# pashtari/factorizer

Measured on AMD Instinct MI355X. Metric: volumes/sec fwd+bwd, Swin Factorizer 128^3, higher is better.
Workload: dtype f32

## Files before the change

factorizer_amd/csrc/gemm.hip:

```cpp
#include "gemm_bx.h"
#include "finish.h"

namespace fz {

__device__ __forceinline__ float half_sum32(float v) {
  v += dpp_take<0xB1, 0xf>(v);
  v += dpp_take<0x4E, 0xf>(v);
  v += dpp_take<0x141, 0xf>(v);
  v += dpp_take<0x140, 0xf>(v);
  v += dpp_take<0x142, 0xa>(v);
  return v;
}

template <int NACC, bool GADD, bool GADD_LDS = false, typename AT = float>
__device__ __forceinline__ void lnbwd_block(const GemmArgsT<AT>& p, const f32x16 (&acc)[NACC], int b, int64_t ncol,
                                            bool col_ok, int lane, int wave, float* red ,
                                            int64_t part_row, const float* g_lds ,
                                            const float* gadd_lds = nullptr ) {
  const int h = lane >> 5;
  const int64_t nc = col_ok ? ncol : 0;
  const unsigned lane_off = (unsigned)(4 * h) * (unsigned)p.Ncol + (unsigned)nc;
  const int64_t sample = (int64_t)b * 32 * p.Ncol;
  const float* sp = p.lnb_stats + (int64_t)b * 2 * p.Ncol;
  float mu[NACC], rs[NACC];
// ... 2540 lines not shown
        s2[e] += src[(MB * NACC * 16 + NACC + e) * 64];
      }
    }
  }

  float mu_d[NACC], rstd[NACC];
  if (PRO == PRO_LN) {
#pragma unroll
    for (int e = 0; e < NACC; ++e) {
      const float t1 = s1[e] + __shfl_xor(s1[e], 32, 64);
      const float t2 = s2[e] + __shfl_xor(s2[e], 32, 64);
      const float inv = 1.0f / (float)p.Cin;
      const float md = t1 * inv;
      float var = t2 * inv - md * md;
      var = var > 0.f ? var : 0.f;
      mu_d[e] = md;
      rstd[e] = 1.0f / sqrtf(var + p.ln_eps);
    }
    if (p.stats_out != nullptr && by == 0 && h == 0 && col_ok) {
      float mean[NACC];
#pragma unroll
      for (int e = 0; e < NACC; ++e) mean[e] = shift[e] + mu_d[e];
      float* so = p.stats_out + (int64_t)b * 2 * p.Vin;
      vstore<NACC>(so + col_off, mean);
      vstore<NACC>(so + p.Vin + col_off, rstd);
    }
  }
  if (!col_ok) return;
  const int64_t ncol = (LOADER == LOAD_S2D) ? n0 + 2 * j : col_off;
#pragma unroll
  for (int mb = 0; mb < MB; ++mb) {
    if (PRO == PRO_LN) {
#pragma unroll
      for (int r = 0; r < 16; ++r) {
        const int rl = (r & 3) + 8 * (r >> 2) + 4 * h;
        const float sw = sW[mb * 32 + rl];
#pragma unroll
        for (int q = 0; q < NACC; ++q) acc[mb][q][r] = rstd[q] * (acc[mb][q][r] - mu_d[q] * sw);
      }
    }
    store_block<NACC, EPI, LOADER == LOAD_S2D>(p, acc[mb], b, m0 + mb * 32, ncol, h,
                                                PRO == PRO_LN ? tW + mb * 32 : nullptr);
  }
}

}

using namespace fz;

static std::atomic<int> g_bx_on{-1};
static int knob_pos(const fz::EnvKnob& k, int dflt) { return k.set && k.val > 0 ? k.val : dflt; }
static int knob_mlp_wg_wgs() { return knob_pos(FZ_KNOB("FZ_MLP_WG_WGS"), 512); }
static int knob_gemm_dw_wgs() { return knob_pos(FZ_KNOB("FZ_GEMM_DW_WGS"), 512); }
static int knob_chain64_p512() { return knob_pos(FZ_KNOB("FZ_CHAIN64_P512"), 1) == 1; }
static int knob_res_prefetch() { return knob_pos(FZ_KNOB("FZ_RES_PREFETCH"), 1) == 1; }
static int knob_p32() { return knob_pos(FZ_KNOB("FZ_GEMM_P32"), 1) == 1; }
static int knob_p32_wgs() { return knob_pos(FZ_KNOB("FZ_GEMM_P32_WGS"), 512); }
static int knob_head_fwd() { const auto& k = FZ_KNOB("FZ_HEAD_FWD"); return k.set ? k.val : 1; }
static int knob_chain_wgb() { const auto& k = FZ_KNOB("FZ_CHAIN_WGB"); return k.set ? k.val : 1; }
static int knob_chain_fwd_bx() { const auto& k = FZ_KNOB("FZ_CHAIN_FWD_BX"); return k.set ? k.val : 1; }
static int knob_mlp_wgs(int dflt) { return knob_pos(FZ_KNOB("FZ_MLP_WGS"), dflt); }

static int gemm_bx_enabled() {
  int v = g_bx_on.load(std::memory_order_relaxed);
  if (v < 0) {
    const char* e = getenv("FZ_GEMM_BX");
    v = e ? (atoi(e) != 0) : 1;
    g_bx_on.store(v, std::memory_order_relaxed);
  }
  return v;
}
extern "C" int fz_gemm_bx_enable(int on) {
  const int prev = gemm_bx_enabled();
  if (on >= 0) g_bx_on.store(on != 0, std::memory_order_relaxed);
  return prev;
}

template <typename AT>
static int gemm_launch(const fz_gemm_desc* d, fz_stream_t stream) {
  if (!d->x[0] || !d->w || !d->y) return fail(FZ_E_ARG, "fz_gemm: null pointer");
  if (d->loader < LOAD_PLAIN || d->loader > LOAD_K3) return fail(FZ_E_ARG, "fz_gemm: bad loader");
  if (d->epilogue < EPI_PLAIN || d->epilogue > EPI_LNBWD) return fail(FZ_E_ARG, "fz_gemm: bad epilogue");
  const bool lnb64 = d->epilogue == EPI_LNBWD && d->M == 64 && d->K == 64 && d->nsrc == 1 && !d->bmul;
  if (d->epilogue == EPI_LNBWD && ((!lnb64 && (d->M != 32 || (d->K != 32 && d->K != 64))) || d->loader != LOAD_PLAIN || !d->lnb_x || !d->lnb_stats ||
                                   !d->lnb_g || !d->lnb_part || d->bias || d->res || d->emul || d->eact || d->ln))
    return fail(FZ_E_UNSUPPORTED, "fz_gemm: LayerNorm-backward epilogue needs M == 32 (K = 32 or 64) or M == K == 64, plain loader");
  if (d->epilogue == EPI_LNBWD && d->Ncol > ((int64_t)1 << 27)) return fail(FZ_E_UNSUPPORTED, "fz_gemm: LayerNorm-backward epilogue: more than 2^27 voxels per sample");
  if (d->B < 0 || d->Cin < 1 || d->M < 1 || d->K < 1) return fail(FZ_E_SHAPE, "fz_gemm: sizes must be positive");
  if ((d->K & 1) && (d->loader != LOAD_PLAIN || d->ln))
    return fail(FZ_E_UNSUPPORTED, "fz_gemm: odd K only with the plain loader and no LayerNorm prologue");
  if (d->loader == LOAD_K3 && (d->epilogue != EPI_PLAIN || d->ln || d->src_mode != 0 || d->nsrc != 1 ||
                               (d->Wi & 3) || d->K != 27 * d->Cin || (d->Cin & 1)))
    return fail(FZ_E_UNSUPPORTED, "fz_gemm: k3 loader needs W % 4 == 0, even Cin, K = 27*Cin, plain epilogue");
  if (d->bmul && (d->loader != LOAD_PLAIN || d->src_mode != 0 || d->nsrc != 1))
    return fail(FZ_E_UNSUPPORTED, "fz_gemm: bmul needs the plain single-source loader");
  if (d->Ncol % 4 != 0 && d->loader != LOAD_S2D) return fail(FZ_E_UNSUPPORTED, "fz_gemm: voxel count must be a multiple of 4");
  if (d->loader == LOAD_S2D && ((d->Wo & 1) || d->epilogue != EPI_PLAIN || d->ln || d->src_mode != 0 || d->nsrc != 1))
    return fail(FZ_E_UNSUPPORTED, "fz_gemm: space-to-depth loader needs even coarse width, plain epilogue");
  if (d->epilogue == EPI_D2S && (d->M % 8 != 0)) return fail(FZ_E_SHAPE, "fz_gemm: depth-to-space rows must be 8*C");
  if (d->nsrc < 1 || d->nsrc > 2 || d->src_mode != 0)
    return fail(FZ_E_UNSUPPORTED, "fz_gemm: one source, or two sources concatenated along channels");
  if (d->bmul && d->bmul_kind != ACT_RELU) return fail(FZ_E_UNSUPPORTED, "fz_gemm: bmul supports the ReLU gate");
  if (d->B == 0) return FZ_OK;
  GemmArgsT<AT> a;
  for (int i = 0; i < 4; ++i) a.x[i] = (const AT*)d->x[i];
  a.nsrc = d->nsrc; a.src_mode = d->src_mode; a.c0 = d->c0 > 0 ? d->c0 : d->Cin; a.Cin = d->Cin;
  a.Vin = d->Vin; a.Di = d->Di; a.Hi = d->Hi; a.Wi = d->Wi; a.bmul = (const AT*)d->bmul; a.bmul_kind = d->bmul_kind;
  a.w = d->w; a.w_t = d->w_t; a.ldw = d->ldw; a.M = d->M; a.K = d->K;
  a.bias = d->bias; a.ln = d->ln; a.ln_g = d->ln_g; a.ln_b = d->ln_b; a.ln_eps = d->ln_eps;
  a.stats_out = d->stats_out; a.bact = d->bact; a.eact = d->eact; a.res = (const AT*)d->res; a.emul = (const AT*)d->emul;
  a.emul_kind = d->emul_kind; a.y = (AT*)d->y; a.Ncol = d->Ncol; a.Ho = d->Ho; a.Wo = d->Wo; a.B = d->B;
  a.dbg = 0; a.tile_map = 1;
  a.ygroups = 0; a.xtiles = 0; a.tune = d->tune;
  a.lnb_x = (const AT*)d->lnb_x; a.lnb_stats = d->lnb_stats; a.lnb_g = d->lnb_g; a.lnb_gadd = (const AT*)d->lnb_gadd; a.lnb_part = d->lnb_part;
  hipStream_t st = (hipStream_t)stream;
  const int mblocks = (d->M + 31) / 32;
  if (lnb64) {
    if (d->Ncol % 4 != 0) return fail(FZ_E_UNSUPPORTED, "fz_gemm: voxel count must be a multiple of 4");
    if (!d->lnb_gadd) return fail(FZ_E_UNSUPPORTED, "fz_gemm: the 64-channel LayerNorm-backward epilogue needs the added gradient");
    ChainArgsT<AT> c = {};
    const int ntiles = (int)fz_mlp_partials(d->B, d->Ncol);
    constexpr int lds64 = (8192 + 8192 + 128 + 64 + 512) * (int)sizeof(float);
    auto kern = products_split(d->products) ? gemm_chain64_kernel<true, AT, true, true> : gemm_chain64_kernel<true, AT, true, false>;
    FZ_HIP_OK(hipFuncSetAttribute(reinterpret_cast<const void*>(kern), hipFuncAttributeMaxDynamicSharedMemorySize, lds64));
    hipLaunchKernelGGL(kern, dim3((unsigned)(ntiles < 512 ? ntiles : 512)), dim3(256), lds64, st, a, c, ntiles);
    FZ_LAUNCH_CHECK();
    return FZ_OK;
  }

  {
    const int bx_on = products_split(d->products);
    const int pro_bx = d->ln ? 1 : (d->bact == ACT_GELU ? 2 : (d->bmul ? 3 : 0));
    const bool one_pro = (d->ln != 0) + (d->bact != 0) + (d->bmul != nullptr) <= 1;
    const int bx_kmin = (sizeof(AT) == 2 && !d->ln && d->bact == 0) ? 32 : 64;
    if (bx_on && one_pro && d->bact != ACT_RELU && d->K >= bx_kmin && d->M >= 32 && (d->loader == LOAD_PLAIN || d->loader == LOAD_S2D) &&
        (d->epilogue == EPI_PLAIN || d->epilogue == EPI_D2S) && !(d->loader == LOAD_S2D && pro_bx) && !(d->epilogue == EPI_D2S && pro_bx))
    {
      const int rc = gemm_bx_launch<AT>(a, d->loader, d->epilogue, pro_bx, stream);
      if (rc != FZ_E_UNSUPPORTED) return rc;
    }
  }

  if (knob_head_fwd() && d->loader == LOAD_PLAIN && d->epilogue == EPI_PLAIN && d->M <= 4 && d->K == 32 && d->Cin == 32 && a.c0 == 32 &&
      !d->ln && !d->bact && !d->eact && !d->res && !d->bmul && !d->emul && !d->w_t && d->ldw == 32 && d->Ncol == d->Vin && d->Ncol % 4 == 0 &&
      d->Ncol / 4 < ((int64_t)1 << 31) && (int64_t)d->B * (d->Ncol / 4) < ((int64_t)1 << 31) && d->stats_out == nullptr)
    return fz_head_fwd(d->x[0], d->w, d->bias, d->y, d->B, d->M, 32, d->Ncol, d->act_dtype, stream);

  if (knob_p32() && d->loader == LOAD_PLAIN && d->epilogue == EPI_PLAIN && d->M <= 32 && d->K == 32 && d->Cin == 32 && (a.c0 & 1) == 0 && d->Vin < ((int64_t)1 << 28) &&
      (int64_t)5 * d->Ncol * (int64_t)sizeof(AT) < ((int64_t)1 << 32)  && !d->res && !d->bmul &&
      !d->emul && d->Ncol % 4 == 0 && d->Ncol == d->Vin && d->B * ((d->Ncol + 127) / 128) >= 4096 && d->B * ((d->Ncol + 127) / 128) < ((int64_t)1 << 30) &&
      !(d->bact && !d->ln) ) {
    const unsigned ntiles = (unsigned)(d->B * ((d->Ncol + 127) / 128));
    const unsigned cap = (unsigned)knob_p32_wgs();
    const unsigned wgs = (ntiles + 3) / 4 < cap ? (ntiles + 3) / 4 : cap;
    const int pf = (d->bact ? 1 : 0) | (d->ln ? 2 : 0);
    dim3 grid(wgs), block(256);
    if (pf == 0) hipLaunchKernelGGL((gemm_p32_kernel<0, AT>), grid, block, 0, st, a, ntiles);
    else if (pf == 2) hipLaunchKernelGGL((gemm_p32_kernel<2, AT>), grid, block, 0, st, a, ntiles);
    else hipLaunchKernelGGL((gemm_p32_kernel<3, AT>), grid, block, 0, st, a, ntiles);
    FZ_LAUNCH_CHECK();
    return FZ_OK;
  }

  int res_maxk = 32;
  if (d->epilogue == EPI_LNBWD) res_maxk = 64;
  const bool stream_small = mblocks == 1 && d->K >= 16 && d->K <= 32 && !d->res && !d->bmul && !d->emul &&
                            d->epilogue == EPI_PLAIN && d->bact == 0;
  if (d->loader == LOAD_PLAIN && d->K <= res_maxk && !stream_small) {
    const int nA = (d->K + 1) / 2;
    int RB = mblocks < 8 ? mblocks : 8;
    while ((size_t)(nA * RB * 64 + 32 * RB) * sizeof(float) > 65536) --RB;
    const size_t lds = (size_t)(nA * RB * 64 + 32 * RB + (d->epilogue == EPI_LNBWD ? 256 : 0)) * sizeof(float);
    const int64_t tiles = (d->Ncol + 511) / 512;
    dim3 grid((unsigned)(tiles * d->B), (unsigned)((mblocks + RB - 1) / RB)), block(256);
#define FZ_RES_PF(NS, E, BM, PFv) hipLaunchKernelGGL((gemm_resident_kernel<NS, E, BM, false, AT, PFv>), grid, block, lds, st, a, RB)
#define FZ_RES(NS, E, BM)                                                  \
  do {                                                                    \
    const int pf = (d->bact ? 1 : 0) | (d->ln ? 2 : 0);                   \
    if (pf == 0) FZ_RES_PF(NS, E, BM, 0);                                 \
    else if (pf == 1) FZ_RES_PF(NS, E, BM, 1);                            \
    else if (pf == 2) FZ_RES_PF(NS, E, BM, 2);                            \
    else FZ_RES_PF(NS, E, BM, 3);                                         \
  } while (0)
    if (d->epilogue == EPI_LNBWD) {
      if (d->bmul) return fail(FZ_E_UNSUPPORTED, "fz_gemm: bmul with LayerNorm-backward epilogue");
#define FZ_RES_LNB(NS, GA) hipLaunchKernelGGL((gemm_resident_kernel<NS, EPI_LNBWD, false, GA>), grid, block, lds, st, a, RB)
      if (d->lnb_gadd) { if (nA <= 16) FZ_RES_LNB(16, true); else FZ_RES_LNB(32, true); }
      else { if (nA <= 16) FZ_RES_LNB(16, false); else FZ_RES_LNB(32, false); }
    } else if (d->epilogue == EPI_D2S) {
      if (d->bmul) return fail(FZ_E_UNSUPPORTED, "fz_gemm: bmul with depth-to-space epilogue");
      if (nA <= 16) FZ_RES(16, EPI_D2S, false); else FZ_RES(32, EPI_D2S, false);
    } else if (d->bmul) {
      if (nA <= 16) FZ_RES(16, EPI_PLAIN, true); else FZ_RES(32, EPI_PLAIN, true);
    } else if (d->res && !d->emul && d->M == 32 && nA <= 16 && !d->ln && knob_res_prefetch()) {
      if (d->bact) hipLaunchKernelGGL((gemm_resident_kernel<16, EPI_PLAIN, false, false, AT, 1, true>), grid, block, lds, st, a, RB);
      else hipLaunchKernelGGL((gemm_resident_kernel<16, EPI_PLAIN, false, false, AT, 0, true>), grid, block, lds, st, a, RB);
    } else {
      if (nA <= 16) FZ_RES(16, EPI_PLAIN, false); else FZ_RES(32, EPI_PLAIN, false);
    }
    FZ_LAUNCH_CHECK();
    return FZ_OK;
  }

  int nacc = 4, MBsel = mblocks >= 2 ? 2 : 1;
  if (d->loader == LOAD_S2D) { nacc = 2; MBsel = 1; }
  else {
    const bool narrow_ok = d->loader == LOAD_PLAIN && d->epilogue == EPI_PLAIN;
    auto wgs = [&](int na, int mb) {
      const int64_t t = (d->Ncol + 32 * na * 4 - 1) / (32 * na * 4);
      return t * d->B * ((mblocks + mb - 1) / mb);
    };
    if (wgs(nacc, MBsel) < 512 && MBsel == 2) MBsel = 1;
    if (narrow_ok) {
      if (wgs(nacc, MBsel) < 256) nacc = 2;
      if (wgs(nacc, MBsel) < 256 && !(wgs(1, MBsel) < 256 && d->K >= 256)) nacc = 1;
      const char* e = FZ_KNOB("FZ_GEMM_CFG").str;
      if (e && e[0] && e[1]) { nacc = e[0] - '0'; MBsel = e[1] - '0'; if (MBsel == 2 && (nacc != 4 || mblocks < 2)) MBsel = 1; }
    }
  }
  const int TN = 32 * nacc;
  int ks = 1;
  {
    const int64_t wg1 = ((d->Ncol + TN * 4 - 1) / (TN * 4)) * d->B * ((mblocks + MBsel - 1) / MBsel);
    const bool shape_ok = MBsel == 1 && ((d->loader == LOAD_PLAIN && d->epilogue == EPI_PLAIN && nacc <= 2) ||
                                         d->loader == LOAD_S2D);
    if (shape_ok && wg1 < 256 && d->K >= 256) ks = 4;
  }
  const int WT = ks > 1 ? 1 : 4;
  const int64_t tiles = (d->Ncol + TN * WT - 1) / (TN * WT);
  const int ygr = (mblocks + MBsel - 1) / MBsel;
  int xcd_grid = 1;
  a.ygroups = (xcd_grid && ygr > 1 && ygr <= 8 && tiles * d->B >= 64) ? ygr : 0;
  a.xtiles = (int)(tiles * d->B);
  dim3 grid((unsigned)(tiles * d->B), (unsigned)ygr), block(256);
  if (a.ygroups > 1) grid = dim3((unsigned)(((tiles * d->B + 7) / 8) * 8 * ygr), 1);
#define FZ_STR(MB, NA, L, E, PR) hipLaunchKernelGGL((gemm_stream_kernel<MB, NA, L, E, PR>), grid, block, 0, st, a)
#define FZ_STRK(MB, NA, L, E, PR) hipLaunchKernelGGL((gemm_stream_kernel<MB, NA, L, E, PR, 4>), grid, block, 0, st, a)
  if (d->bact == ACT_RELU) return fail(FZ_E_UNSUPPORTED, "fz_gemm: ReLU input prologue is not compiled (streaming)");
  const int pro = d->ln ? PRO_LN : (d->bact == ACT_GELU ? PRO_GELU : (d->bmul ? PRO_BMUL : PRO_NONE));
  if ((d->ln != 0) + (d->bact != 0) + (d->bmul != nullptr) > 1)
    return fail(FZ_E_UNSUPPORTED, "fz_gemm: at most one input prologue (LayerNorm / GELU / gate)");
  if (d->loader == LOAD_S2D) { if (ks == 4) FZ_STRK(1, 2, LOAD_S2D, EPI_PLAIN, PRO_NONE); else FZ_STR(1, 2, LOAD_S2D, EPI_PLAIN, PRO_NONE); }
  else if (d->loader == LOAD_K3) { if (MBsel == 2) FZ_STR(2, 4, LOAD_K3, EPI_PLAIN, PRO_NONE); else FZ_STR(1, 4, LOAD_K3, EPI_PLAIN, PRO_NONE); }
  else if (d->epilogue == EPI_D2S) {
    if (pro != PRO_NONE) return fail(FZ_E_UNSUPPORTED, "fz_gemm: prologue with depth-to-space epilogue");
    if (MBsel == 2) FZ_STR(2, 4, LOAD_PLAIN, EPI_D2S, PRO_NONE); else FZ_STR(1, 4, LOAD_PLAIN, EPI_D2S, PRO_NONE);
  } else {
#define FZ_STR_SHAPES(PR)                                                                                   \
  do {                                                                                                      \
    if (nacc == 4) { if (MBsel == 2) FZ_STR(2, 4, LOAD_PLAIN, EPI_PLAIN, PR); else FZ_STR(1, 4, LOAD_PLAIN, EPI_PLAIN, PR); } \
    else if (nacc == 2) { if (ks == 4) FZ_STRK(1, 2, LOAD_PLAIN, EPI_PLAIN, PR); else FZ_STR(1, 2, LOAD_PLAIN, EPI_PLAIN, PR); } \
    else { if (ks == 4) FZ_STRK(1, 1, LOAD_PLAIN, EPI_PLAIN, PR); else FZ_STR(1, 1, LOAD_PLAIN, EPI_PLAIN, PR); } \
  } while (0)
    if (pro == PRO_LN) FZ_STR_SHAPES(PRO_LN);
    else if (pro == PRO_GELU) FZ_STR_SHAPES(PRO_GELU);
    else if (pro == PRO_BMUL) FZ_STR_SHAPES(PRO_BMUL);
    else FZ_STR_SHAPES(PRO_NONE);
  }
  FZ_LAUNCH_CHECK();
  return FZ_OK;
}

extern "C" int fz_gemm(const fz_gemm_desc* d, fz_stream_t stream) {
  if (!d) return fail(FZ_E_ARG, "fz_gemm: null descriptor");
  if (d->act_dtype == FZ_STORE_F32) return gemm_launch<float>(d, stream);
  if (d->act_dtype == FZ_STORE_BF16) return gemm_launch<bf16>(d, stream);
  return fail(FZ_E_ARG, "fz_gemm: act_dtype must be FZ_STORE_F32 or FZ_STORE_BF16");
}

extern "C" int64_t fz_gemm_lnbwd_partials(const fz_gemm_desc* d) {
  if (!d) return -1;
  if (d->M == 64) return fz_mlp_partials(d->B, d->Ncol);
  return ((d->Ncol + 511) / 512) * d->B;
}

static int mlp_nacc() { return 2; }

extern "C" int64_t fz_mlp_partials(int B, int64_t V) {
  const int64_t tw = 128 * mlp_nacc();
  return ((V + tw - 1) / tw) * (int64_t)B;
}

extern "C" int fz_mlp_wgrad_rows(int B, int64_t V) {
  const int64_t nt = fz_mlp_partials(B, V);
  const int wgs = knob_mlp_wg_wgs();
  return (int)(nt < wgs ? nt : wgs);
}
extern "C" int64_t fz_mlp_wgrad_workspace_bytes(int B, int64_t V) {
  return 2 * (int64_t)fz_mlp_wgrad_rows(B, V) * kWgRow * (int64_t)sizeof(float);
}

extern "C" int fz_mlp_pre_supported(int C, int H, int64_t V, int products) {
  if (!(V > 0 && (V % 4) == 0 && V <= ((int64_t)1 << 27) && products_split(products))) return 0;
  if (C == 32 && H == 64) return knob_chain_fwd_bx() ? 1 : 0;
  if (C == 64 && H == 128) return (((V + 255) / 256) % 2 == 0 && knob_chain64_p512()) ? 1 : 0;
  return 0;
}

extern "C" int fz_mlp_supported(int C, int H, int64_t V) {
  const bool shape = (C == 32 && (H == 64 || H == 128)) || (C == 64 && H == 128);
  return (shape && V > 0 && (V % 4) == 0 && V <= ((int64_t)1 << 27)) ? 1 : 0;
}

template <typename AT>
static int mlp_launch(const fz_mlp_desc* d, fz_stream_t stream) {
  if (!fz_mlp_supported(d->C, d->H, d->V)) return fail(FZ_E_UNSUPPORTED, "fz_mlp_chain: needs (C, H) in {(32, 64), (32, 128), (64, 128)}, V % 4 == 0");
  if (d->C == 64 && d->mode == 2) return fail(FZ_E_UNSUPPORTED, "fz_mlp_chain: the fused weight gradients need C == 32, H == 64");
  if (d->B < 0) return fail(FZ_E_SHAPE, "fz_mlp_chain: negative batch");
  const bool pre = d->pre_in != nullptr;
  if (pre && (d->mode != 0 || !d->pre_w || !d->pre_res || !d->pre_out))
    return fail(FZ_E_ARG, "fz_mlp_chain: pre_in needs mode 0, pre_w, pre_res, pre_out (see fz_mlp_pre_supported)");
  if (pre && !fz_mlp_pre_supported(d->C, d->H, d->V, d->products))
    return fail(FZ_E_UNSUPPORTED, "fz_mlp_chain: the fused out-projection runs on split-bf16 products only (fz_mlp_pre_supported)");
  if (d->post_out && (!pre || d->C != 32 || !d->post_w || d->post_m < 1 || d->post_m > 4))
    return fail(FZ_E_ARG, "fz_mlp_chain: post_out needs pre_in, C == 32, post_w and 1 <= post_m <= 4");
  if ((!d->in && !pre) || !d->w1 || !d->w2 || !d->out || !d->z1 || !d->stats)
    return fail(FZ_E_ARG, "fz_mlp_chain: null pointer");
  if (d->mode == 0 && (!d->ln_g || !d->ln_b)) return fail(FZ_E_ARG, "fz_mlp_chain: forward needs the LayerNorm affine");
  if (d->mode == 1 && (!d->gz1 || !d->x1 || !d->ln_g || !d->part)) return fail(FZ_E_ARG, "fz_mlp_chain: backward needs gz1, x1, gamma, part");
  if (d->mode == 2 && (!d->x1 || !d->ln_g || !d->ln_b || !d->gln || !d->wpart || !d->gw1 || !d->gb1 || !d->gw2 || !d->gb2))
    return fail(FZ_E_ARG, "fz_mlp_chain: backward with weight gradients needs x1, gamma, beta, gln, wpart, gw1, gb1, gw2, gb2");
  if (d->mode == 2 && d->H == 128 && !d->glp) return fail(FZ_E_ARG, "fz_mlp_chain: the fused weight gradients at H == 128 need the glp buffer");
  if (d->mode < 0 || d->mode > 2) return fail(FZ_E_ARG, "fz_mlp_chain: bad mode");
  if (d->B == 0) {
    if (d->mode == 2) {
      hipStream_t s0 = (hipStream_t)stream;
      FZ_HIP_OK(hipMemsetAsync(d->gw1, 0, sizeof(float) * d->H * 32, s0));
      FZ_HIP_OK(hipMemsetAsync(d->gw2, 0, sizeof(float) * d->H * 32, s0));
      FZ_HIP_OK(hipMemsetAsync(d->gb1, 0, sizeof(float) * d->H, s0));
      FZ_HIP_OK(hipMemsetAsync(d->gb2, 0, sizeof(float) * 32, s0));
      FZ_HIP_OK(hipMemsetAsync(d->gln, 0, sizeof(float) * 64, s0));
    }
    return FZ_OK;
  }
  GemmArgsT<AT> a = {};
  ChainArgsT<AT> c = {};
  a.x[0] = (const AT*)d->in; a.nsrc = 1; a.c0 = 32; a.Cin = 32; a.Vin = d->V; a.M = d->H; a.K = 32; a.Ncol = d->V; a.B = d->B;
  hipStream_t st = (hipStream_t)stream;
  const int ntiles = (int)fz_mlp_partials(d->B, d->V);
  if (d->C == 64) {
    if (d->mode == 1 && !d->in) return fail(FZ_E_ARG, "fz_mlp_chain: null pointer");
    a.x[0] = (const AT*)d->in; a.nsrc = 1; a.c0 = 64; a.Cin = 64; a.Vin = d->V; a.M = 128; a.K = 64; a.Ncol = d->V; a.B = d->B;
    const int wgs64 = knob_mlp_wgs(512);
    dim3 grid64((unsigned)(ntiles < wgs64 ? ntiles : wgs64));
    constexpr int lds64 = (8192 + 8192 + 128 + 64 + 512) * (int)sizeof(float);
    constexpr int lds512 = (12288 + 12288 + 128 + 64 + 1024) * (int)sizeof(float);
    const bool p512 = products_split(d->products) && ntiles % 2 == 0 && knob_chain64_p512();
    dim3 grid512((unsigned)(ntiles / 2 < 256 ? ntiles / 2 : 256));
    if (d->mode == 0) {
      a.w = d->w1; a.w_t = 0; a.ldw = 64;
      a.bias = d->b1; a.ln = 1; a.ln_g = d->ln_g; a.ln_b = d->ln_b; a.ln_eps = d->ln_eps; a.stats_out = d->stats;
      a.res = (const AT*)d->in; a.y = (AT*)d->out;
      c.wB = d->w2; c.wB_t = 0; c.ldwB = 128; c.biasB = d->b2; c.side = (AT*)d->z1;
      if (pre) {
        if (!p512) return fail(FZ_E_UNSUPPORTED, "fz_mlp_chain: the fused out-projection at C == 64 needs an even number of tiles");
// ... 164 lines not shown
```

factorizer_amd/csrc/gemm_bx.h:

```cpp
#pragma once
#include "gemm_common.h"

namespace fz {

typedef __bf16 bx8 __attribute__((ext_vector_type(8)));
typedef __bf16 bx2 __attribute__((ext_vector_type(2)));
typedef float fx2 __attribute__((ext_vector_type(2)));

enum { BXPRO_NONE = 0, BXPRO_LN = 1, BXPRO_GELU = 2, BXPRO_BMUL = 3 };

template <int NT>
__device__ __forceinline__ void bx_split(const float (&x)[8], bx8 (&t)[NT]) {
#pragma unroll
  for (int i = 0; i < 8; i += 2) {
    fx2 v = {x[i], x[i + 1]};
    const bx2 a = __builtin_convertvector(v, bx2);
    t[0][i] = a[0]; t[0][i + 1] = a[1];
    if constexpr (NT >= 2) {
      v = v - __builtin_convertvector(a, fx2);
      const bx2 b = __builtin_convertvector(v, bx2);
      t[1][i] = b[0]; t[1][i + 1] = b[1];
      if constexpr (NT >= 3) {
        v = v - __builtin_convertvector(b, fx2);
        const bx2 c = __builtin_convertvector(v, bx2);
// ... 108 lines not shown
#pragma unroll
    for (int mb = 0; mb < MB; ++mb) {
      const int64_t urow = (int64_t)b * p.M + m0 + mb * 32;
      constexpr int RBT = NACC == 4 ? 4 : (NACC == 2 ? 8 : 16);
#pragma unroll
      for (int r0 = 0; r0 < 16; r0 += RBT) {
      float ev[RBT][NACC], rv[RBT][NACC];
      if (p.emul != nullptr) {
#pragma unroll
        for (int rr = 0; rr < RBT; ++rr) uload<NACC>(p.emul + (urow + ((r0 + rr) & 3) + 8 * ((r0 + rr) >> 2)) * p.Ncol, yoff, ev[rr]);
      }
      if (p.res != nullptr) {
#pragma unroll
        for (int rr = 0; rr < RBT; ++rr) uload<NACC>(p.res + (urow + ((r0 + rr) & 3) + 8 * ((r0 + rr) >> 2)) * p.Ncol, yoff, rv[rr]);
      }
#pragma unroll
      for (int rr = 0; rr < RBT; ++rr) {
        const int r = r0 + rr;
        const int rl = (r & 3) + 8 * (r >> 2) + 4 * h;
        float add = sBias[mb * 32 + rl];
        float v[NACC];
        if (LN) {
          const float sw = sW[mb * 32 + rl];
          add += tW[mb * 32 + rl];
#pragma unroll
          for (int q = 0; q < NACC; ++q) v[q] = rstd[q] * (acc[mb][q][r] - mu_d[q] * sw) + add;
        } else {
#pragma unroll
          for (int q = 0; q < NACC; ++q) v[q] = acc[mb][q][r] + add;
        }
        if (p.eact) {
#pragma unroll
          for (int q = 0; q < NACC; ++q) v[q] = act_f(p.eact, v[q]);
        }
        if (p.emul != nullptr) {
#pragma unroll
          for (int q = 0; q < NACC; ++q) v[q] *= act_grad_f(p.emul_kind, ev[rr][q]);
        }
        if (p.res != nullptr) {
#pragma unroll
          for (int q = 0; q < NACC; ++q) v[q] += rv[rr][q];
        }
        AT* yp = reinterpret_cast<AT*>(reinterpret_cast<char*>(p.y + (urow + (r & 3) + 8 * (r >> 2)) * p.Ncol) + yoff);
        vstore<NACC>(yp, v);
      }
      }
    }
  } else {
    const int Wf = 2 * p.Wo, Hf = 2 * p.Ho;
    const int64_t Vf = 8 * p.Ncol;
    const int Mo = p.M >> 3;
    const int wo = (int)(col_off % p.Wo);
    const int64_t t2 = col_off / p.Wo;
    const int ho = (int)(t2 % p.Ho);
    const int dz = (int)(t2 / p.Ho);
    const unsigned foff = (unsigned)((((int64_t)(2 * dz + h) * Hf + 2 * ho) * Wf + 2 * wo) * ES);
#pragma unroll
    for (int mb = 0; mb < MB; ++mb) {
      const int64_t uo = (int64_t)b * Mo + ((m0 + mb * 32) >> 3);
      float rv[8][2 * NACC];
      if (p.res != nullptr) {
#pragma unroll
        for (int rp = 0; rp < 8; ++rp)
          uload<2 * NACC>(p.res + (uo + (rp >> 1)) * Vf + (int64_t)(rp & 1) * Wf, foff, rv[rp]);
      }
#pragma unroll
      for (int rp = 0; rp < 8; ++rp) {
        const int r0 = 2 * rp;
        const float bs = sBias[mb * 32 + 8 * (rp >> 1)];
        float v[2 * NACC];
#pragma unroll
        for (int q = 0; q < NACC; ++q) { v[2 * q] = acc[mb][q][r0] + bs; v[2 * q + 1] = acc[mb][q][r0 + 1] + bs; }
        if (p.res != nullptr) {
#pragma unroll
          for (int i = 0; i < 2 * NACC; ++i) v[i] += rv[rp][i];
        }
        AT* yp = reinterpret_cast<AT*>(reinterpret_cast<char*>(p.y + (uo + (rp >> 1)) * Vf + (int64_t)(rp & 1) * Wf) + foff);
        vstore<2 * NACC>(yp, v);
      }
    }
  }
}

template <typename AT>
int gemm_bxk_launch(const GemmArgsT<AT>& a, int loader, int epilogue, int pro, int nacc, int mb, fz_stream_t stream);

}
```

factorizer_amd/pointwise.py:

```python
from __future__ import annotations

import ctypes
import os
import threading as _threading
import weakref

import torch
import torch.nn.functional as F

from . import _native as N
from . import gradbuf as _GB
from . import functional as Fn

ACT = {"none": 0, "relu": 1, "gelu": 2}
LOAD_PLAIN, LOAD_S2D, LOAD_K3 = 0, 1, 2
EPI_PLAIN, EPI_D2S = 0, 1


def _p(t):
    return None if t is None else t.data_ptr()


def _vox(x):
    v = 1
# ... 19 lines not shown
    d.stats_out = _p(stats_out)
    d.bact, d.bmul, d.bmul_kind = bact, _p(bmul), bmul_kind
    d.eact, d.res, d.emul, d.emul_kind = eact, _p(res), _p(emul), emul_kind
    d.y, d.Ncol, d.Ho, d.Wo, d.B = _p(y), Ncol, Ho, Wo, B
    d.loader, d.epilogue = loader, epilogue
    x0 = xs[0]
    d.act_dtype = N.act_dtype(x0)
    nbytes = x0.element_size() * (sum(t.numel() for t in xs) + y.numel() + (res.numel() if res is not None else 0))
    with torch.cuda.device(x0.device):
        rc = Fn._timed(f"{name}_{Cin}->{M}", nbytes,
                       lambda: N.lib().fz_gemm(ctypes.byref(d), N.stream_ptr(x0)),
                       cols=B * max(Vin, Ncol * (8 if epilogue == EPI_D2S else 1)), flops=2 * B * Ncol * M * K)
    N.check(rc, "fz_gemm")
    return y


def _wgrad_desc(p, qs, gw, *, B, M, Cin, K, Vq, Ncols, gbias=None, pmul=None, pmul_kind=0, src_mode=0, c0=0,
                stats=None, qact=0, ln=None, loader=0, D=0, H=0, W=0, Ho=0, Wo=0, accumulate=False, name="wgrad"):
    d = N.WgradDesc()
    d.products = N.products()
    d.p, d.M, d.pmul, d.pmul_kind = _p(p), M, _p(pmul), pmul_kind
    for i in range(4):
        d.q[i] = _p(qs[i]) if i < len(qs) else None
    d.nsrc, d.src_mode, d.c0, d.Cin, d.K, d.Vq = len(qs), src_mode, c0, Cin, K, Vq
    d.D, d.H, d.W, d.N, d.Ho, d.Wo = D, H, W, Ncols, Ho, Wo
    d.stats, d.qact = _p(stats), qact
    if ln is not None:
        d.ln_g, d.ln_b = _p(ln[0]), _p(ln[1])
    d.gw, d.gbias, d.accumulate, d.B, d.loader = _p(gw), _p(gbias), int(accumulate), B, loader
    d.act_dtype = N.act_dtype(p)
    nb = N.lib().fz_wgrad_workspace_bytes(ctypes.byref(d))
    if nb < 0:
        raise N.NativeError("fz_wgrad_workspace_bytes failed")
    ws = torch.empty(max(nb // 4, 1), dtype=torch.float32, device=p.device)
    nbytes = p.element_size() * (p.numel() + sum(t.numel() for t in qs))
    return d, ws, f"{name}_{M}x{K}", nbytes, B * max(Vq, Ncols), 2 * B * Ncols * M * K


def _wgrad(p, qs, gw, **kw):
    d, ws, key, nbytes, cols, flops = _wgrad_desc(p, qs, gw, **kw)
    with torch.cuda.device(p.device), _finish_scope(ws, gw, kw.get("gbias")):
        rc = Fn._timed(key, nbytes, lambda: N.lib().fz_wgrad(ctypes.byref(d), ws.data_ptr(), N.stream_ptr(p)),
                       cols=cols, flops=flops)
    N.check(rc, "fz_wgrad")
    return gw


_WGRAD_GROUP = os.environ.get("FZ_WGRAD_GROUP", "1") != "0"


def _wgrad_group(problems, name):
    plans = [_wgrad_desc(p, qs, gw, **kw) for p, qs, gw, kw in problems]
    n = len(plans)
    descs = (ctypes.POINTER(N.WgradDesc) * n)(*[ctypes.pointer(pl[0]) for pl in plans])
    wss = (ctypes.c_void_p * n)(*[pl[1].data_ptr() for pl in plans])
    t0 = problems[0][0]
    held = [pl[1] for pl in plans] + [pr[2] for pr in problems] + [pr[3].get("gbias") for pr in problems]
    with torch.cuda.device(t0.device), _finish_scope(*held):
        rc = Fn._timed(name, sum(pl[3] for pl in plans),
                       lambda: N.lib().fz_wgrad_group(descs, wss, n, N.stream_ptr(t0)),
                       cols=max(pl[4] for pl in plans), flops=sum(pl[5] for pl in plans))
    N.check(rc, "fz_wgrad_group")


def _ln_backward(gl, x, stats, ln_w, gadd=None):
    B, C = x.shape[:2]
    V = _vox(x)
    gx = torch.empty_like(x)
    gpar = torch.empty(2 * C, dtype=torch.float32, device=x.device)
    ws = torch.empty(max(N.lib().fz_ln_bwd_workspace_bytes2(B, C, V) // 4, 1), dtype=torch.float32, device=x.device)
    with torch.cuda.device(x.device), _finish_scope(ws, gpar):
        rc = Fn._timed(f"ln_bwd_{C}", 3 * x.element_size() * x.numel(), lambda: N.lib().fz_ln_bwd(
            gl.data_ptr(), x.data_ptr(), stats.data_ptr(), ln_w.data_ptr(), _p(gadd), gx.data_ptr(), _p(gpar), _p(ws),
            B, C, V, N.act_dtype(x), N.stream_ptr(x)), cols=B * V)
    N.check(rc, "fz_ln_bwd")
    return gx, gpar[:C], gpar[C:]


def _dgrad_lnbwd(gz, w2, x, stats, ln_w, gadd):
    B, C = x.shape[:2]
    V = _vox(x)
    Mz = gz.shape[1]
    fused64 = C == 64 and Mz == 64 and gadd is not None and V % 4 == 0 and os.environ.get("FZ_LNBWD64", "1") != "0"
    if not fused64 and (C != 32 or Mz > 64 or Mz % 2):
        gl = torch.empty_like(x)
        _gemm([gz], w2, gl, B=B, Cin=Mz, Vin=V, M=C, K=Mz, Ncol=V, w_t=True, ldw=C, name="linear_dgrad")
        return _ln_backward(gl, x, stats, ln_w, gadd=gadd)
    gx = torch.empty_like(x)
    d = N.GemmDesc()
    d.products = N.products()
    d.x[0] = gz.data_ptr()
    d.nsrc, d.src_mode, d.c0, d.Cin, d.Vin = 1, 0, 0, Mz, V
    d.w, d.w_t, d.ldw, d.M, d.K = w2.data_ptr(), 1, C, C, Mz
    d.y, d.Ncol, d.B = gx.data_ptr(), V, B
    d.loader, d.epilogue = LOAD_PLAIN, 2
    d.lnb_x, d.lnb_stats, d.lnb_g, d.lnb_gadd = x.data_ptr(), stats.data_ptr(), ln_w.data_ptr(), _p(gadd)
    d.act_dtype = N.act_dtype(x)
    rows = N.lib().fz_gemm_lnbwd_partials(ctypes.byref(d))
    part = torch.empty((rows, 2 * C), dtype=torch.float32, device=x.device)
    d.lnb_part = part.data_ptr()
    gpar = torch.empty(2 * C, dtype=torch.float32, device=x.device)
    tmp = torch.empty((64, 2 * C), dtype=torch.float32, device=x.device)
    nbytes = x.element_size() * (gz.numel() + 2 * x.numel() + (gadd.numel() if gadd is not None else 0))
    with torch.cuda.device(x.device):
        rc = Fn._timed(f"dgrad_lnbwd_{Mz}->{C}", nbytes, lambda: N.lib().fz_gemm(ctypes.byref(d), N.stream_ptr(x)),
                       cols=B * V, flops=2 * B * V * C * Mz)
        N.check(rc, "fz_gemm")
        with _finish_scope(part, gpar, tmp):
            rc = N.lib().fz_reduce_rows(part.data_ptr(), rows, 2 * C, gpar.data_ptr(), tmp.data_ptr(), N.stream_ptr(x))
        N.check(rc, "fz_reduce_rows")
    return gx, gpar[:C], gpar[C:]


def _dw_fused_ok(C, V):
    return C == 32 and V % 4 == 0 and V <= (1 << 27) and os.environ.get("FZ_DW_FUSED", "1") != "0"


def _gemm_dw(g, w2, q, ln=None, stats=None, gadd=None, want_bias=False, name="dgrad_wgrad", gw_out=None, gb_out=None):
    B, C = q.shape[:2]
    V = _vox(q)
    dev = q.device
    y = torch.empty_like(q)
    gw = _GB.out_like(w2, (C, C), torch.float32) if gw_out is None else gw_out
    gb = (gb_out if gb_out is not None else torch.empty(C, dtype=torch.float32, device=dev)) if want_bias else None
    wpart = torch.empty(N.lib().fz_gemm_dw_workspace_bytes(B, V) // 4, dtype=torch.float32, device=dev)
    d = N.GemmDwDesc()
    d.g, d.q, d.w, d.y = g.data_ptr(), q.data_ptr(), w2.data_ptr(), y.data_ptr()
    d.wpart, d.gw, d.gb = wpart.data_ptr(), gw.data_ptr(), _p(gb)
    d.B, d.C, d.V, d.act_dtype = B, C, V, N.act_dtype(q)
    d.ldgw = gw.stride(0)
    d.ldw = w2.stride(0)
    gpar = None
    if ln is not None:
        gpar = torch.empty(64, dtype=torch.float32, device=dev)
        d.ln, d.stats, d.ln_g, d.ln_b, d.gadd, d.gln = 1, stats.data_ptr(), ln[0].data_ptr(), ln[1].data_ptr(), _p(gadd), gpar.data_ptr()
    nbytes = q.element_size() * (3 * q.numel() + (gadd.numel() if gadd is not None else 0))
    with torch.cuda.device(dev), _finish_scope(wpart, gw, gb, gpar):
        rc = Fn._timed(f"{name}_{C}", nbytes, lambda: N.lib().fz_gemm_dw(ctypes.byref(d), N.stream_ptr(q)),
                       cols=B * V, flops=4 * B * V * C * C)
        N.check(rc, "fz_gemm_dw")
    if ln is not None:
        return y, gw, gb, gpar[:32], gpar[32:]
    return y, gw, gb, None, None


def _mlp_chain_ok(C, Hd, V):
    return os.environ.get("FZ_MLP_CHAIN", "1") != "0" and bool(N.lib().fz_mlp_supported(C, Hd, V))


def _mlp_fwd_chain(x1, ln_w, ln_b, eps, w12, b1, w22, b2):
    B, C = x1.shape[:2]
    V = _vox(x1)
    Hd = w12.shape[0]
    z1 = torch.empty((B, Hd, *x1.shape[2:]), dtype=x1.dtype, device=x1.device)
    st = torch.empty((B, 2, V), dtype=torch.float32, device=x1.device)
    x2 = torch.empty_like(x1)
    d = N.MlpDesc()
    d.products = N.products()
    d.mode, d.inp, d.w1, d.w2, d.b1, d.b2 = 0, x1.data_ptr(), w12.data_ptr(), w22.data_ptr(), _p(b1), _p(b2)
    d.ln_g, d.ln_b, d.ln_eps = ln_w.data_ptr(), ln_b.data_ptr(), float(eps)
    d.stats, d.z1, d.out = st.data_ptr(), z1.data_ptr(), x2.data_ptr()
    d.B, d.C, d.H, d.V = B, C, Hd, V
    d.act_dtype = N.act_dtype(x1)
    with torch.cuda.device(x1.device):
        rc = Fn._timed(f"mlp_chain_fwd_{C}", x1.element_size() * (2 * x1.numel() + z1.numel()),
                       lambda: N.lib().fz_mlp_chain(ctypes.byref(d), N.stream_ptr(x1)), cols=B * V, flops=4 * B * V * C * Hd)
    N.check(rc, "fz_mlp_chain")
# ... 1146 lines not shown
```

Before: 126.2.

## Fuse linear dgrad with LayerNorm backward for 128/256-channel stages

Adds a kernel that computes the linear-layer data gradient with split-bf16 MFMA and applies the LayerNorm backward epilogue in the same pass, writing per-block gamma/beta partials. The target is 128- and 256-channel stages, which previously ran a separate dgrad GEMM into a temporary followed by a standalone LayerNorm-backward kernel. Fusing removes that temporary's write and re-read plus one launch. The cost is a fixed-shape kernel with register-heavy accumulators and a simple double-buffered weight pipeline, and it only runs for fp32 storage with split products.

```diff
diff --git a/factorizer_amd/csrc/gemm.hip b/factorizer_amd/csrc/gemm.hip
--- a/factorizer_amd/csrc/gemm.hip
+++ b/factorizer_amd/csrc/gemm.hip
@@ -2646,9 +2646,14 @@
   if (d->loader < LOAD_PLAIN || d->loader > LOAD_K3) return fail(FZ_E_ARG, "fz_gemm: bad loader");
   if (d->epilogue < EPI_PLAIN || d->epilogue > EPI_LNBWD) return fail(FZ_E_ARG, "fz_gemm: bad epilogue");
   const bool lnb64 = d->epilogue == EPI_LNBWD && d->M == 64 && d->K == 64 && d->nsrc == 1 && !d->bmul;
-  if (d->epilogue == EPI_LNBWD && ((!lnb64 && (d->M != 32 || (d->K != 32 && d->K != 64))) || d->loader != LOAD_PLAIN || !d->lnb_x || !d->lnb_stats ||
+  const bool lnbdeep = d->epilogue == EPI_LNBWD && (d->M == 128 || d->M == 256);
+  if (d->epilogue == EPI_LNBWD && ((!lnb64 && !lnbdeep && (d->M != 32 || (d->K != 32 && d->K != 64))) || d->loader != LOAD_PLAIN || !d->lnb_x || !d->lnb_stats ||
                                    !d->lnb_g || !d->lnb_part || d->bias || d->res || d->emul || d->eact || d->ln))
-    return fail(FZ_E_UNSUPPORTED, "fz_gemm: LayerNorm-backward epilogue needs M == 32 (K = 32 or 64) or M == K == 64, plain loader");
+    return fail(FZ_E_UNSUPPORTED, "fz_gemm: LayerNorm-backward epilogue needs M == 32 (K = 32 or 64), M == K == 64 or M = 128 / 256, plain loader");
+  if (lnbdeep && (!lnbwd_bx_ok(d->M, d->K, d->Ncol, d->Vin, d->act_dtype, products_split(d->products)) || d->nsrc != 1 ||
+                  d->Cin != d->K || (d->c0 > 0 && d->c0 != d->Cin) || !d->w_t || d->ldw != d->M || d->bmul || d->bact || !d->lnb_gadd))
+    return fail(FZ_E_UNSUPPORTED, "fz_gemm: the LayerNorm-backward epilogue at M = 128 / 256 needs K = 128 / 256 (M = 128) or K = 256 (M = 256), fp32 storage, split-bf16 "
+                                  "products, a transposed (K, M) weight, the added gradient and a voxel count that is a multiple of 8192 / M");
   if (d->epilogue == EPI_LNBWD && d->Ncol > ((int64_t)1 << 27)) return fail(FZ_E_UNSUPPORTED, "fz_gemm: LayerNorm-backward epilogue: more than 2^27 voxels per sample");
   if (d->B < 0 || d->Cin < 1 || d->M < 1 || d->K < 1) return fail(FZ_E_SHAPE, "fz_gemm: sizes must be positive");
   if ((d->K & 1) && (d->loader != LOAD_PLAIN || d->ln))
@@ -2679,6 +2684,10 @@
   a.lnb_x = (const AT*)d->lnb_x; a.lnb_stats = d->lnb_stats; a.lnb_g = d->lnb_g; a.lnb_gadd = (const AT*)d->lnb_gadd; a.lnb_part = d->lnb_part;
   hipStream_t st = (hipStream_t)stream;
   const int mblocks = (d->M + 31) / 32;
+  if (lnbdeep) {
+    if constexpr (sizeof(AT) == 4) return lnbwd_bx_launch(a, stream);
+    else return fail(FZ_E_UNSUPPORTED, "fz_gemm: the LayerNorm-backward epilogue at M = 128 / 256 needs fp32 storage");
+  }
   if (lnb64) {
     if (d->Ncol % 4 != 0) return fail(FZ_E_UNSUPPORTED, "fz_gemm: voxel count must be a multiple of 4");
     if (!d->lnb_gadd) return fail(FZ_E_UNSUPPORTED, "fz_gemm: the 64-channel LayerNorm-backward epilogue needs the added gradient");
@@ -2835,6 +2844,7 @@
 extern "C" int64_t fz_gemm_lnbwd_partials(const fz_gemm_desc* d) {
   if (!d) return -1;
   if (d->M == 64) return fz_mlp_partials(d->B, d->Ncol);
+  if (d->M == 128 || d->M == 256) return lnbwd_bx_rows(d->M, d->B, d->Ncol);
   return ((d->Ncol + 511) / 512) * d->B;
 }
 
diff --git a/factorizer_amd/csrc/gemm_bx.h b/factorizer_amd/csrc/gemm_bx.h
--- a/factorizer_amd/csrc/gemm_bx.h
+++ b/factorizer_amd/csrc/gemm_bx.h
@@ -214,6 +214,10 @@
   }
 }
 
+bool lnbwd_bx_ok(int C, int K, int64_t Ncol, int64_t Vin, int act_dtype, bool split);
+int64_t lnbwd_bx_rows(int C, int B, int64_t Ncol);
+int lnbwd_bx_launch(const GemmArgsT<float>& a, fz_stream_t stream);
+
 template <typename AT>
 int gemm_bxk_launch(const GemmArgsT<AT>& a, int loader, int epilogue, int pro, int nacc, int mb, fz_stream_t stream);
 
diff --git a/factorizer_amd/csrc/lnbwd_bx.hip b/factorizer_amd/csrc/lnbwd_bx.hip
--- /dev/null
+++ b/factorizer_amd/csrc/lnbwd_bx.hip
@@ -0,0 +1,193 @@
+#include "gemm_bx.h"
+
+namespace fz {
+
+__device__ __forceinline__ float lnb_half_sum32(float v) {
+  v += dpp_take<0xB1, 0xf>(v);
+  v += dpp_take<0x4E, 0xf>(v);
+  v += dpp_take<0x141, 0xf>(v);
+  v += dpp_take<0x140, 0xf>(v);
+  v += dpp_take<0x142, 0xa>(v);
+  return v;
+}
+
+template <int C>
+__global__ __launch_bounds__(256, C == 128 ? 2 : 1) void lnbwd_bx_kernel(GemmArgsT<float> p) {
+  constexpr int NTA = 3, NTB = 3;
+  constexpr int WR = C / 64;
+  constexpr int NT = 4 / WR;
+  constexpr int RBK = C / 32;
+  constexpr int CH = 2;
+  constexpr int IPT = CH * RBK * 64 / 256;
+  constexpr int kBuf = CH * RBK * NTA * 64 * 8;
+  static_assert(C == 128 || C == 256, "LayerNorm width 128 or 256");
+  __shared__ __attribute__((aligned(16))) __bf16 As[2 * kBuf];
+  __shared__ float sG[C];
+  __shared__ float sRed[4][2][32];
+  __shared__ float sPart[NT][2 * C];
+
+  const int lane = threadIdx.x & 63;
+  const int wave = __builtin_amdgcn_readfirstlane(threadIdx.x >> 6);
+  const int j = lane & 31, h = lane >> 5;
+  const int ct = wave / WR, rp = wave % WR;
+  const int64_t N = p.Ncol;
+  const int tiles = (int)(N / (32 * NT));
+  const int b = blockIdx.x / tiles;
+  const int64_t col = (int64_t)(blockIdx.x % tiles) * (32 * NT) + 32 * ct + j;
+  const int nG = p.K >> 4;
+
+  for (int i = threadIdx.x; i < C; i += 256) sG[i] = p.lnb_g[i];
+
+  const float* gcol = p.x[0] + ((int64_t)b * p.K + 8 * h) * N + col;
+  auto fetch = [&](int g, float (&s)[8]) {
+    g = g < nG ? g : nG - 1;
+#pragma unroll
+    for (int e = 0; e < 8; ++e) s[e] = gcol[(int64_t)(16 * g + e) * N];
+  };
+  float ring[CH][8];
+#pragma unroll
+  for (int i = 0; i < CH; ++i) fetch(i, ring[i]);
+
+  float wraw[IPT][8];
+  auto load_chunk = [&](int g0) {
+#pragma unroll
+    for (int u = 0; u < IPT; ++u) {
+      const int idx = threadIdx.x + 256 * u;
+      const int l = idx & 63, rbg = idx >> 6;
+      const int m = (rbg % RBK) * 32 + (l & 31);
+      const float* wp = p.w + (int64_t)(16 * (g0 + rbg / RBK) + 8 * (l >> 5)) * p.ldw + m;
+#pragma unroll
+      for (int e = 0; e < 8; ++e) wraw[u][e] = wp[(int64_t)e * p.ldw];
+    }
+  };
+  auto store_chunk = [&](int buf) {
+#pragma unroll
+    for (int u = 0; u < IPT; ++u) {
+      const int idx = threadIdx.x + 256 * u;
+      const int l = idx & 63, rbg = idx >> 6;
+      bx8 t[NTA];
+      bx_split<NTA>(wraw[u], t);
+#pragma unroll
+      for (int i = 0; i < NTA; ++i) *reinterpret_cast<bx8*>(&As[buf * kBuf + ((rbg * NTA + i) * 64 + l) * 8]) = t[i];
+    }
+  };
+
+  f32x16 acc[2];
+#pragma unroll
+  for (int mb = 0; mb < 2; ++mb)
+#pragma unroll
+    for (int r = 0; r < 16; ++r) acc[mb][r] = 0.f;
+
+  load_chunk(0);
+  store_chunk(0);
+  __syncthreads();
+  int cbuf = 0;
+  for (int g0 = 0; g0 < nG; g0 += CH) {
+    const bool more = g0 + CH < nG;
+    if (more) load_chunk(g0 + CH);
+#pragma unroll
+    for (int gl = 0; gl < CH; ++gl) {
+      bx8 bop[NTB];
+      bx_split<NTB>(ring[gl], bop);
+      fetch(g0 + gl + CH, ring[gl]);
+#pragma unroll
+      for (int mb = 0; mb < 2; ++mb) {
+        const int rbg = gl * RBK + 2 * rp + mb;
+        bx8 aop[NTA];
+#pragma unroll
+        for (int i = 0; i < NTA; ++i) aop[i] = *reinterpret_cast<const bx8*>(&As[cbuf * kBuf + ((rbg * NTA + i) * 64 + lane) * 8]);
+        bx_mfma<NTA, NTB>(acc[mb], aop, bop);
+      }
+    }
+    if (more) {
+      store_chunk(cbuf ^ 1);
+      cbuf ^= 1;
+      __syncthreads();
+    }
+  }
+
+  const float* sp = p.lnb_stats + (int64_t)b * 2 * N + col;
+  const float mu = sp[0], rs = sp[N];
+  const int64_t rowoff = ((int64_t)b * C + 64 * rp + 4 * h) * N + col;
+  float xh[2][16], ga[2][16];
+#pragma unroll
+  for (int mb = 0; mb < 2; ++mb)
+#pragma unroll
+    for (int r = 0; r < 16; ++r) {
+      const int64_t o = rowoff + (int64_t)(32 * mb + (r & 3) + 8 * (r >> 2)) * N;
+      xh[mb][r] = p.lnb_x[o];
+      ga[mb][r] = p.lnb_gadd[o];
+    }
+  float m1 = 0.f, m2 = 0.f;
+#pragma unroll
+  for (int mb = 0; mb < 2; ++mb)
+#pragma unroll
+    for (int r = 0; r < 16; ++r) {
+      const int row = 64 * rp + 32 * mb + (r & 3) + 8 * (r >> 2) + 4 * h;
+      xh[mb][r] = (xh[mb][r] - mu) * rs;
+      const float gv = acc[mb][r] * sG[row];
+      m1 += gv;
+      m2 += gv * xh[mb][r];
+    }
+  m1 += __shfl_xor(m1, 32, 64);
+  m2 += __shfl_xor(m2, 32, 64);
+  if (h == 0) {
+    sRed[wave][0][j] = m1;
+    sRed[wave][1][j] = m2;
+  }
+  __syncthreads();
+  m1 = 0.f;
+  m2 = 0.f;
+#pragma unroll
+  for (int w = 0; w < WR; ++w) {
+    m1 += sRed[ct * WR + w][0][j];
+    m2 += sRed[ct * WR + w][1][j];
+  }
+  m1 *= 1.0f / (float)C;
+  m2 *= 1.0f / (float)C;
+
+  float* yp = p.y + rowoff;
+#pragma unroll
+  for (int mb = 0; mb < 2; ++mb)
+#pragma unroll
+    for (int r = 0; r < 16; ++r) {
+      const int rl = 32 * mb + (r & 3) + 8 * (r >> 2);
+      const int row = 64 * rp + rl + 4 * h;
+      const float v = rs * (acc[mb][r] * sG[row] - m1 - xh[mb][r] * m2) + ga[mb][r];
+      yp[(int64_t)rl * N] = v;
+      const float sg = lnb_half_sum32(acc[mb][r] * xh[mb][r]);
+      const float sb = lnb_half_sum32(acc[mb][r]);
+      if (j == 31) {
+        sPart[ct][row] = sg;
+        sPart[ct][C + row] = sb;
+      }
+    }
+  __syncthreads();
+  float* part = p.lnb_part + (int64_t)blockIdx.x * 2 * C;
+  for (int e = threadIdx.x; e < 2 * C; e += 256) {
+    float s = 0.f;
+#pragma unroll
+    for (int c = 0; c < NT; ++c) s += sPart[c][e];
+    part[e] = s;
+  }
+}
+
+int64_t lnbwd_bx_rows(int C, int B, int64_t Ncol) { return (int64_t)B * (Ncol / (32 * (256 / C))); }
+
+bool lnbwd_bx_ok(int C, int K, int64_t Ncol, int64_t Vin, int act_dtype, bool split) {
+  if (C != 128 && C != 256) return false;
+  if (K != C && !(C == 128 && K == 256)) return false;
+  if (act_dtype != FZ_STORE_F32 || !split) return false;
+  return Vin == Ncol && Ncol > 0 && Ncol % (32 * (256 / C)) == 0;
+}
+
+int lnbwd_bx_launch(const GemmArgsT<float>& a, fz_stream_t stream) {
+  hipStream_t st = (hipStream_t)stream;
+  const dim3 grid((unsigned)lnbwd_bx_rows(a.M, a.B, a.Ncol)), block(256);
+  if (a.M == 128) hipLaunchKernelGGL(lnbwd_bx_kernel<128>, grid, block, 0, st, a);
+  else hipLaunchKernelGGL(lnbwd_bx_kernel<256>, grid, block, 0, st, a);
+  FZ_LAUNCH_CHECK();
+  return FZ_OK;
+}
+
+}
diff --git a/factorizer_amd/pointwise.py b/factorizer_amd/pointwise.py
--- a/factorizer_amd/pointwise.py
+++ b/factorizer_amd/pointwise.py
@@ -125,7 +125,10 @@
     V = _vox(x)
     Mz = gz.shape[1]
     fused64 = C == 64 and Mz == 64 and gadd is not None and V % 4 == 0 and os.environ.get("FZ_LNBWD64", "1") != "0"
-    if not fused64 and (C != 32 or Mz > 64 or Mz % 2):
+    split = N.products() == N.PRODUCTS_SPLIT_BF16 or (N.products() == N.PRODUCTS_DEFAULT and N.lib().fz_gemm_bx_enable(-1) != 0)
+    fused_deep = (C in (128, 256) and (Mz == C or (C, Mz) == (128, 256)) and gadd is not None and x.dtype == torch.float32 and split
+                  and V % (8192 // C) == 0 and os.environ.get("FZ_LNBWD_DEEP", "1") != "0")
+    if not fused64 and not fused_deep and (C != 32 or Mz > 64 or Mz % 2):
         gl = torch.empty_like(x)
         _gemm([gz], w2, gl, B=B, Cin=Mz, Vin=V, M=C, K=Mz, Ncol=V, w_t=True, ldw=C, name="linear_dgrad")
         return _ln_backward(gl, x, stats, ln_w, gadd=gadd)
```

Measured after the change: 126.1 (median of 6 runs). No clear change (-0.1%).
